# dselivanov/rsparse

Hardware: AMD Instinct MI355X
Metric: als_iterations_per_sec (higher is better)
Workload: dtype f32 (Gram products of rows > 512 / <= 32 non-zeros as 2 x fp16 / 3 x bf16 split terms of the fp32 operands, fp32 accumulate; everything else fp32); 1 GPU; WRMF implicit ALS, CG(3), synthetic 10000000x1000000, 500155883 nnz, rank 128, lambda 0.1; survey_config=3, feedback=implicit, n_items=1000000, nnz=500155883, rank=128, solver=conjugate_gradient, cg_steps=3, parallelism=rows sharded x1, factors replicated

## Files before the change

rsparse_amd/build.py:

```python
import subprocess
import sys
import time
from concurrent.futures import ThreadPoolExecutor
from pathlib import Path

PKG = Path(__file__).resolve().parent
CSRC = PKG / "csrc"
SRC = [CSRC / n for n in ("wrmf_kernels.hip", "wrmf_cgq.hip", "wrmf_cgp.hip", "wrmf_ne.hip", "wrmf_chol.hip", "wrmf_chol_wave.hip", "wrmf_chol_mf.hip", "wrmf_cg_mf.hip", "wrmf_chol_lr.hip",
                          "wrmf_topk.hip", "wrmf_topk_large.hip", "wrmf_similar.hip", "wrmf_metrics.hip", "wrmf_ingest.hip", "wrmf_nnls.hip", "wrmf_bias.hip", "wrmf_lu.hip",
                          "wrmf_f64.hip", "wrmf_wide.hip", "wrmf_wide_cg.hip", "wrmf_ctx_kernels.hip", "wrmf_schedule.cpp", "wrmf_capi.cpp", "wrmf_f64_capi.cpp", "wrmf_ctx.cpp")]
HEADERS = [CSRC / "wrmf_chol_mf.attrs.csv", CSRC / "wrmf_mf.h", CSRC / "wrmf_internal.h", CSRC / "wrmf_capi_common.h", CSRC / "wrmf_schedule.h", CSRC / "wrmf_device.h", CSRC / "wrmf_wave.h", CSRC / "wrmf_ldlt.h", CSRC / "wrmf_f64.h", PKG.parent / "include" / "rsparse_wrmf_hip.h"]
DEPS = SRC + HEADERS
OUT = PKG / "lib" / "librsparse_wrmf_hip.so"
FLAGS = ["--offload-arch=gfx950", "-O3", "-std=c++17", "-fPIC"]


EXTRA_FLAGS = {n: ["-mllvm", "-forceattrs-csv-path=" + str(CSRC / "wrmf_chol_mf.attrs.csv"), "-fno-slp-vectorize"] for n in ("wrmf_chol_mf.hip", "wrmf_cg_mf.hip")}
AUDITED = {"wrmf_chol_mf.hip", "wrmf_cg_mf.hip"}
REG_LIMIT = {"wrmf_cg_mf.hip": 512}


def audit_listing(src, extra, obj):
    sys.path.insert(0, str(PKG.parent / "tools" / "dbg"))
    import acc_audit
    lst = obj.with_suffix(".s")

    def listing(flags, floor):
        cmd = ["hipcc", *FLAGS, *flags, "-S", "--cuda-device-only", str(src), "-o", str(lst)]
        r = subprocess.run(cmd, stdout=subprocess.PIPE, stderr=subprocess.PIPE, text=True)
        if r.returncode != 0:
            raise RuntimeError("hipcc -S failed on %s:\n%s" % (src.name, r.stderr[-3000:]))
        acc, flight, _ = acc_audit.audit(str(lst), quiet=True, acc_floor=floor)
        return acc, flight, lst.read_text()
    acc, flight, text = listing(extra, 0)
# ... 23 lines not shown
    src = [s for s in SRC if s.exists()]
    hdr_m = max(h.stat().st_mtime for h in HEADERS)
    todo, objs = [], []
    for s in src:
        o = objdir / (s.stem + ".o")
        objs.append(o)
        if force or not o.exists() or o.stat().st_mtime < max(s.stat().st_mtime, hdr_m):
            todo.append((s, o))
    if not todo and out.exists() and all(out.stat().st_mtime >= o.stat().st_mtime for o in objs):
        return out

    def compile_one(so):
        s, o = so
        t0 = time.time()
        extra = EXTRA_FLAGS.get(s.name, [])
        cmd = ["hipcc", *FLAGS, *extra, "-c", str(s), "-o", str(o)]
        r = subprocess.run(cmd, stdout=subprocess.PIPE, stderr=subprocess.PIPE, text=True)
        if r.returncode != 0:
            raise RuntimeError("hipcc failed on %s:\n%s" % (s.name, r.stderr[-6000:]))
        if s.name in AUDITED:
            audit_listing(s, extra, o)
        if verbose:
            print("  %-20s %.1f s" % (s.name, time.time() - t0), flush=True)

    with ThreadPoolExecutor(max_workers=8) as ex:
        list(ex.map(compile_one, todo))
    cmd = ["hipcc", "--offload-arch=gfx950", "-fPIC", "-shared", *map(str, objs), "-ldl", "-lpthread", "-o", str(out)]
    subprocess.check_call(cmd)
    return out


if __name__ == "__main__":
    argv = sys.argv[1:]
    outp = argv[argv.index("--out") + 1] if "--out" in argv else None
# ... 3 lines not shown
```

rsparse_amd/csrc/wrmf_capi.cpp:

```cpp
#include "../../include/rsparse_wrmf_hip.h"

#include <cxxabi.h>

#include <algorithm>
#include <cfloat>
#include <cmath>
#include <cstdlib>
#include <cstring>
#include <string>
#include <vector>

#include "wrmf_capi_common.h"

using namespace rsparse_hip;

struct rsparse_hip_csc {
  DevCSC d;
  int device = 0;
  std::vector<void*> owned;
};

namespace {
thread_local std::string g_err;
}
// ... 119 lines not shown
}

int build_schedule(rsparse_hip_csc& m, const int32_t* host_col_ptrs) {
  DevCSC& d = m.d;
  int cus = 256;
  HIP_TRY(hipDeviceGetAttribute(&cus, hipDeviceAttributeMultiprocessorCount, m.device));
  d.q_cfg = cgq_default_cfg();
  SchedulePlan plan;
  if (!plan_schedule(host_col_ptrs, d.n_cols, cus, [](int len) { return cgq_bucket_of(len, cgq_default_cfg()); }, plan))
    return fail(RSPARSE_HIP_ERR_INVALID, "col_ptrs is not non-decreasing");
  d.max_len = plan.max_len; d.nnz_long = plan.nnz_long; d.n_empty = plan.n_empty;
  d.short_max = kTileNnz; d.n_long = plan.n_long;
  for (int b = 0; b < 7; b++) d.q_off[b] = plan.off[b];
  for (int b = 0; b < 6; b++) d.q_nnz[b] = plan.nnz[b];
  d.q_pair_first = plan.pair_first; d.q_team4_first = plan.team4_first;
  d.q_gt32 = plan.gt32; d.q_gt48 = plan.gt48; d.q_lr_first = plan.lr_first; d.q_n_lr = plan.n_lr;
  d.q_n_chol_long = plan.n_chol_long; d.q_n_nec = plan.n_nec;
  int rc;
  if ((rc = upload(m, plan.order, &d.q_order))) return rc;
  if ((rc = upload(m, plan.stream_off, &d.q_stream_off))) return rc;
  if ((rc = upload_cut(m, plan.cut, d.q_ne))) return rc;
  d.q_ne1 = d.q_ne;
  if ((rc = upload_deal(m, plan.fine, d.q_ne))) return rc;
  if ((rc = upload_deal(m, plan.coarse, d.q_ne1))) return rc;
  if (plan.nec_is_ne) {
    d.q_nec = d.q_ne;
  } else {
    if ((rc = upload_cut(m, plan.cut_nec, d.q_nec))) return rc;
    if ((rc = upload_deal(m, plan.nec, d.q_nec))) return rc;
  }
// ... 119 lines not shown
    hipError_t we = wave_cg ? launch_wide_cg_wave(a, implicit, kWideCgMaxLen, d.max_len > kWideCgMaxLen ? d.q_order : nullptr, 0, s)
                            : launch_als_wide(a, implicit, solver, g_ws.wide_m2, g_ws.wide_lu, s);
    if (we != hipSuccess) return hip_fail(we, wave_cg ? "launch_wide_cg_wave" : "launch_als_wide");
    if ((we = launch_sum_partials(g_ws.partials, wave_cg ? (size_t)grid_w : (size_t)grid, outw, s, g_ws.partials + g_ws.partial_slots())) != hipSuccess)
      return hip_fail(we, "launch_sum_partials");
    return RSPARSE_HIP_OK;
  }
  const bool cg = solver == RSPARSE_SOLVER_CONJUGATE_GRADIENT;
  const bool cgq = cg && use_cgq(rank, d_X, d_Y);
  QSchedule qs;
  qs.order = d.q_order;
  qs.cfg = d.q_cfg;
  qs.pair_first = d.q_pair_first;
  for (int b = 0; b < 7; b++) qs.off[b] = d.q_off[b];
  qs.team4_first = (implicit && bias && bias->gbias != 0.f) ? d.q_off[2] : d.q_team4_first;
  qs.pair_wide = cgp_wide_supported(rank, implicit, implicit && bias && bias->gbias != 0.f);
  const bool cg_mf = cgq && implicit && !bias && cg_mf_supported(rank, implicit) && d.q_order && d.q_off[1] > d.q_n_nec;
  if (cg_mf) {
    qs.mf_rows = d.q_order + d.q_n_nec;
    qs.mf_n = d.q_off[1] - d.q_n_nec;
  }
  const bool chol_mf = chol_mf_supported(rank) && !cg && solver == RSPARSE_SOLVER_CHOLESKY && !bias && d.q_order && ne_supported(rank) &&
                       use_cgq(rank, d_X, d_Y) && d.q_lr_first > d.q_off[1];
  const int mf_first = d.q_off[1];
  const int n_mf = chol_mf ? d.q_lr_first - mf_first : 0;
  const bool nec_lists = padded_rank(rank) > 64 && d.q_nec.wg > 0 && !chol_mf;
  const bool ne_chol = !cg && solver == RSPARSE_SOLVER_CHOLESKY && !bias && (nec_lists || d.q_ne.wg > 0 || chol_mf) &&
                       ne_supported(rank) && use_cgq(rank, d_X, d_Y);
  qs.ne = (cg_mf || (ne_chol && nec_lists)) ? d.q_nec : ((implicit && padded_rank(rank) == 128) ? d.q_ne : d.q_ne1);
  const size_t chol_base = chol2_loss_slots(d.n_cols);
// ... 1048 lines not shown
```

rsparse_amd/csrc/wrmf_cgq.hip:

```cpp
#include <algorithm>

#include "wrmf_internal.h"
#include "wrmf_device.h"

namespace rsparse_hip {
namespace {

using namespace dev;

constexpr int kGvFirstMinCapq = 16;
constexpr int kStreamPrefixQ = 4;
constexpr int kIdxPrefetchMaxWpr = 2;

constexpr int kMaxSavedSweeps = 4;

template <int KP>
struct QG {
  static constexpr int RPN = KP / 16;
  static constexpr int VW = RPN >= 4 ? 4 : RPN;
  static constexpr int NV = RPN / VW;
  __device__ static __forceinline__ int elem(int i, int r) { return (r / VW) * (16 * VW) + i * VW + (r % VW); }
};

template <int VW>
struct Piece;
template <>
struct Piece<4> { using type = float4; };
template <>
struct Piece<2> { using type = float2; };

__device__ __forceinline__ float groups_reduce_scatter4(const float a0, const float a1, const float a2, const float a3) {
  const auto s01 = __builtin_amdgcn_permlane16_swap(__float_as_uint(a0), __float_as_uint(a1), false, false);
  const float c = __uint_as_float(s01[0]) + __uint_as_float(s01[1]);
  const auto s23 = __builtin_amdgcn_permlane16_swap(__float_as_uint(a2), __float_as_uint(a3), false, false);
  const float d = __uint_as_float(s23[0]) + __uint_as_float(s23[1]);
  const auto t = __builtin_amdgcn_permlane32_swap(__float_as_uint(c), __float_as_uint(d), false, false);
  return __uint_as_float(t[0]) + __uint_as_float(t[1]);
}
template <int KP, int CAPQ, int WAVES, int WPR, int STREAM, bool IMPLICIT, int DMF = 0>
struct QSmem {
  static constexpr size_t gram_floats = (IMPLICIT && DMF != 1) ? (size_t)KP * KP : 0;
  static constexpr size_t vec_floats = IMPLICIT ? (size_t)WAVES * KP : 0;
  static constexpr size_t red_floats = WPR > 1 ? (size_t)2 * WAVES * KP + 2 * WAVES : 0;
  static constexpr bool cv_lds = !STREAM && CAPQ * (KP / 16) > 128;
  static constexpr size_t tsv_floats = (STREAM && !IMPLICIT) ? 0 : (size_t)WAVES * (cv_lds ? 3 : 2) * CAPQ * 4;
  static constexpr size_t pre_floats = STREAM ? (size_t)WAVES * kStreamPrefixQ * 4 * KP : 0;
  static constexpr int dmf_ps = KP + 8, dmf_os = KP + 4;
  static constexpr size_t dmf_floats = DMF ? (size_t)WAVES * dmf_ps + (size_t)WAVES * dmf_os : 0;
  static constexpr size_t pfx_floats =
      (!STREAM && WPR > kIdxPrefetchMaxWpr && (CAPQ == 16 || CAPQ == 20)) ? (size_t)WAVES * 2 * CAPQ * 4 : 0;
  static constexpr size_t wl_floats = cv_lds ? (size_t)WAVES * 2 : 0;
  static constexpr size_t xs_floats = cv_lds ? (size_t)WAVES * KP : 0;
  static constexpr size_t bytes =
      (gram_floats + vec_floats + red_floats + tsv_floats + pre_floats + dmf_floats + pfx_floats + wl_floats + xs_floats) * 4 + 16;
};

template <int KP, int CAPQ, int WAVES, int WPR, int STREAM, bool IMPLICIT, int DMF = 0, bool GB = false, bool KFULL = false>
__global__ __launch_bounds__(WAVES * 64, 2) void als_cgq_kernel(AlsArgs a, const int32_t* __restrict__ rows, int n_rows,
                                                             int rows_per_team, size_t loss_slot0) {
  using G_ = QG<KP>;
  constexpr int RPN = G_::RPN, VW = G_::VW, NV = G_::NV, CAP = CAPQ * 4, TEAMS = WAVES / WPR;
  using piece_t = typename Piece<VW>::type;
  using SM = QSmem<KP, CAPQ, WAVES, WPR, STREAM, IMPLICIT, DMF>;
  static_assert(WAVES % WPR == 0, "teams must tile the workgroup");
  constexpr bool GRS = RPN == 8 && VW == 4;
// ... 96 lines not shown
          split_f16(g0 * gs, g1 * gs, hi[e / 2], lo[e / 2]);
        }
        const uint4 h4 = {hi[0], hi[1], hi[2], hi[3]}, l4 = {lo[0], lo[1], lo[2], lo[3]};
        if constexpr (DMF == 1) {
          gAh[t][ks] = __builtin_bit_cast(f16x8, h4);
          gAl[t][ks] = __builtin_bit_cast(f16x8, l4);
        } else {
          *reinterpret_cast<uint4*>(sGf + ((t * 4 + ks) * 2 + 0) * 1024 + lane * 16) = h4;
          *reinterpret_cast<uint4*>(sGf + ((t * 4 + ks) * 2 + 1) * 1024 + lane * 16) = l4;
        }
      }
    if constexpr (DMF == 2) wave_sync();
  }
  float* vec = sVec + wv * KP;
  constexpr bool CVLDS = SM::cv_lds;
  float* tacc = sTsv + wv * (CVLDS ? 3 : 2) * CAP;
  float* tcur = tacc + CAP;
  float* csv = tcur + CAP;
  int buf = 0;
  double wloss = 0.0;
  double* wl_lds = reinterpret_cast<double*>(sPfx + SM::pfx_floats) + wv;
  if (CVLDS && lane == 0) *wl_lds = 0.0;
  float* xs = sPfx + SM::pfx_floats + SM::wl_floats + wv * KP;
  int pf_id = 0, pf_cnt = -1;
  float pf_c = 0.f;
  const int team_global = blockIdx.x * TEAMS + team;
  const int total_teams = gridDim.x * TEAMS;

  auto row_index = [&](int itn) { return team_global + itn * total_teams; };
  int row_c = 0, p1_c = 0, p2_c = 0, row_n = 0;
  if (rows_per_team > 0 && row_index(0) < n_rows) {
    row_c = rows[row_index(0)];
    p1_c = a.col_ptrs[row_c];
    p2_c = a.col_ptrs[row_c + 1];
  }
  if (rows_per_team > 1 && row_index(1) < n_rows) row_n = rows[row_index(1)];
  for (int it = 0; it < rows_per_team; ++it) {
    const int ri = row_index(it);
    const bool have = ri < n_rows;
    if (WPR == 1 && !DMF && !have) break;
    const int row = have ? rfl(row_c) : 0;
    const int p1 = have ? rfl(p1_c) : 0;
    const int p2 = have ? rfl(p2_c) : 0;
    {
      int p1_n = 0, p2_n = 0, row_nn = 0;
      if (it + 1 < rows_per_team && row_index(it + 1) < n_rows) {
        p1_n = a.col_ptrs[row_n];
        p2_n = a.col_ptrs[row_n + 1];
      }
      if (it + 2 < rows_per_team && row_index(it + 2) < n_rows) row_nn = rows[row_index(it + 2)];
      row_c = row_n;
      p1_c = p1_n;
      p2_c = p2_n;
      row_n = row_nn;
    }
    const int cnt = p2 - p1;
    float* yrow = a.Y + (size_t)row * k;
    if (!GB && WPR == 1 && cnt <= 0) {
      if (!DMF || have)
        for (int e = lane; e < k; e += 64) yrow[e] = 0.f;
      if constexpr (!DMF) continue;
    }
    constexpr int PQ = STREAM ? kStreamPrefixQ : 0, PCAP = PQ * 4, PTEAM = PCAP * WPR;
    const int pre = STREAM ? min(cnt, PTEAM) : 0;
    const int pw = STREAM ? max(0, min(PCAP, pre - tw * PCAP)) : 0;
    const int nchunks = (cnt - pre + CAP - 1) / CAP;
    constexpr bool resident = STREAM == 0;
    const float lam_use =
        IMPLICIT ? 0.f : (float)(a.lambda_loss * (a.dynamic_lambda ? (double)(float)cnt : 1.0));

    float* tscr = nullptr;
    float alph[kMaxSavedSweeps];
#pragma unroll
    for (int s2 = 0; s2 < kMaxSavedSweeps; s2++) alph[s2] = 0.f;
    if constexpr (STREAM == 1) {
      if (a.tscr && have && a.cg_steps <= kMaxSavedSweeps) tscr = a.tscr + a.stream_off[ri];
    }

    float xt[CAPQ][RPN];
    float cv[CVLDS ? 1 : CAPQ];
    constexpr int NSL = (CAP + 63) / 64;
    float cl[CVLDS ? 1 : NSL];
#pragma unroll
    for (int s2 = 0; s2 < (CVLDS ? 1 : NSL); s2++) cl[s2] = 0.f;
    auto csv_fill = [&](auto&& conf_of, const int n) {
#pragma unroll
      for (int s2 = 0; s2 < NSL; s2++) {
        const int sl = lane + 64 * s2;
        if (s2 == 0 || sl < CAP) csv[(sl & 3) * CAPQ + (sl >> 2)] = sl < n ? conf_of(sl) : 0.f;
      }
    };
    int ccnt = 0;

    constexpr bool ZPAD = STREAM == 0;
    constexpr bool TSAVE = STREAM == 0;
    constexpr bool GVFIRST = STREAM == 0 && CAPQ >= kGvFirstMinCapq;
    constexpr bool IDXPF = CAP <= 64 && ((STREAM == 0 && WPR <= kIdxPrefetchMaxWpr) || (STREAM == 1 && IMPLICIT));
    constexpr bool DMAPF = KFULL && !IDXPF && SM::pfx_floats > 0;
    int* pfxI = reinterpret_cast<int*>(sPfx) + wv * 2 * CAP;
    float* pfxC = sPfx + wv * 2 * CAP + CAP;
    auto dma_slot = [&](const int j0, const int n) {
      const int j = j0 + min(lane, n - 1);
      dma4(a.row_idx + j, lds_addr(pfxI));
      dma4(a.vals + j, lds_addr(pfxC));
      if constexpr (CAP > 64) {
        if (lane < CAP - 64) {
          const int j2 = j0 + min(lane + 64, n - 1);
          dma4(a.row_idx + j2, lds_addr(pfxI + 64));
          dma4(a.vals + j2, lds_addr(pfxC + 64));
        }
      }
    };
    int pf_pos = -1;
    auto gather_q = [&](auto nq_tag, const int base, const int n, const bool from_pf = false) {
      constexpr int NQG = decltype(nq_tag)::value;
      int id[NQG > 0 ? NQG : 1];
      if constexpr (DMAPF) {
        if (!from_pf && n > 0) {
          dma_slot(base, n);
          wait_vm<0>();
        }
        wave_sync();
#pragma unroll
        for (int q = 0; q < NQG; q++) {
          const int j = max(min(4 * q + g, n - 1), 0);
          id[q] = pfxI[j];
          if constexpr (!CVLDS) cv[q] = (!ZPAD || 4 * q + g < n) ? pfxC[j] : 0.f;
        }
        if constexpr (CVLDS) {
          csv_fill([&](int sl) { return pfxC[sl]; }, n);
        } else if constexpr (TSAVE) {
#pragma unroll
          for (int s2 = 0; s2 < NSL; s2++) cl[s2] = lane + 64 * s2 < n ? pfxC[min(lane + 64 * s2, CAP - 1)] : 0.f;
        }
        wave_sync();
      } else if (IDXPF && from_pf) {
        int* xi = reinterpret_cast<int*>(tacc);
        wave_sync();
        xi[lane & (CAP - 1)] = pf_id;
        tcur[lane & (CAP - 1)] = pf_c;
        wave_sync();
#pragma unroll
        for (int q = 0; q < NQG; q++) {
          const int j = max(min(4 * q + g, n - 1), 0);
          id[q] = xi[j];
          if constexpr (!CVLDS) cv[q] = (!ZPAD || 4 * q + g < n) ? tcur[j] : 0.f;
        }
        if constexpr (TSAVE) cl[0] = lane < n ? pf_c : 0.f;
        wave_sync();
      } else {
#pragma unroll
        for (int q = 0; q < NQG; q++) {
          const int j = max(min(4 * q + g, n - 1), 0);
          id[q] = a.row_idx[base + j];
          if constexpr (!CVLDS) {
            const float c = a.vals[base + j];
            cv[q] = (!ZPAD || 4 * q + g < n) ? c : 0.f;
          }
        }
        if constexpr (CVLDS) {
          wave_sync();
          csv_fill([&](int sl) { return a.vals[base + sl]; }, n);
          wave_sync();
        } else if constexpr (TSAVE) {
#pragma unroll
          for (int s2 = 0; s2 < NSL; s2++) cl[s2] = lane + 64 * s2 < n ? a.vals[base + lane + 64 * s2] : 0.f;
        }
      }
#pragma unroll
      for (int q = 0; q < NQG; q++) {
        const float* src = (!ZPAD || 4 * q + g < n) ? a.X + (size_t)id[q] * k : a.zero_row;
#pragma unroll
        for (int b = 0; b < NV; b++) {
          const int off = b * 16 * VW + i * VW;
          if constexpr (KFULL) {
            const piece_t pc = *reinterpret_cast<const piece_t*>(src + off);
            const float* pf = reinterpret_cast<const float*>(&pc);
#pragma unroll
            for (int c = 0; c < VW; c++) xt[q][b * VW + c] = pf[c];
          } else {
            const piece_t pc = *reinterpret_cast<const piece_t*>(src + min(off, k - VW));
            const float* pf = reinterpret_cast<const float*>(&pc);
#pragma unroll
            for (int c = 0; c < VW; c++) xt[q][b * VW + c] = off < k ? pf[c] : 0.f;
          }
        }
      }
    };
    auto gather = [&](const int base, const int n, const bool from_pf = false) {
      gather_q(std::integral_constant<int, CAPQ>{}, base, n, from_pf);
    };
    float* pre_lds = sPre + (size_t)wv * PQ * 4 * KP + g * KP;
    auto prefix_chunk = [&](const bool first) {
      if constexpr (PQ > 0) {
        const int base = p1 + tw * PCAP;
        if (first) {
          gather_q(std::integral_constant<int, PQ>{}, base, pw);
#pragma unroll
          for (int q = 0; q < PQ; q++)
#pragma unroll
            for (int b = 0; b < NV; b++) {
              piece_t pc;
              float* pf = reinterpret_cast<float*>(&pc);
// ... 218 lines not shown
                  const float* pf = reinterpret_cast<const float*>(&pc);
#pragma unroll
                  for (int c = 0; c < VW; c++) acc[b * VW + c] = fmaf(vv[u], pf[c], acc[b * VW + c]);
                }
              }
            }
          }
        };
        if constexpr (GVFIRST) dense_part();
        if (resident) {
          if (mode != 2 || !TSAVE) {
            quad_pass(v, mode, acc, lacc, nullptr);
          } else {
            wave_sync();
            float esum = 0.f;
#pragma unroll
            for (int s2 = 0; s2 < NSL; s2++) {
              const int sl = NSL == 1 ? (lane & (CAP - 1)) : min(lane + 64 * s2, CAP - 1);
              const float t = tacc[sl];
              const float clv = CVLDS ? csv[(sl & 3) * CAPQ + (sl >> 2)] : cl[s2];
              const float d = IMPLICIT ? ltgt - t : clv - t;
              const float e = IMPLICIT ? clv * d * d : d * d;
              esum += lane + 64 * s2 < ccnt ? e : 0.f;
            }
            lacc = row16_sum(esum);
          }
        } else if (mode == 2 && tscr) {
          for (int ch = tw; ch < (cnt + CAP - 1) / CAP; ch += WPR) {
            const int n = min(CAP, cnt - ch * CAP);
            if (lane < n) {
              const size_t pos = (size_t)ch * CAP + lane;
              float t = tscr[pos];
#pragma unroll
              for (int s2 = 0; s2 < kMaxSavedSweeps; s2++)
                if (s2 < a.cg_steps) t = fmaf(alph[s2], tscr[(size_t)(s2 + 1) * a.stream_nnz + pos], t);
              const float c = a.vals[p1 + pos];
              const float d = IMPLICIT ? ltgt - t : c - t;
              lacc += IMPLICIT ? c * d * d : d * d;
// ... 135 lines not shown
    float dummy = 0.f;
    sweep(x, 0, r, dummy, live);
    auto x_piece = [&](const int b) { return reinterpret_cast<piece_t*>(xs + b * 16 * VW + i * VW); };
    if constexpr (CVLDS) {
      if (g == 0) {
#pragma unroll
        for (int b = 0; b < NV; b++) {
          piece_t pc;
          float* pf = reinterpret_cast<float*>(&pc);
#pragma unroll
          for (int c = 0; c < VW; c++) pf[c] = x[b * VW + c];
          *x_piece(b) = pc;
        }
      }
    }
    if constexpr (IDXPF && STREAM == 0) {
      if (it + 1 < rows_per_team && row_index(it + 1) < n_rows) {
        const int np1 = rfl(p1_c), ncnt = rfl(p2_c) - np1;
        const int nper = min(CAP, (((ncnt + WPR - 1) / WPR) + 15) & ~15);
        const int ncc = max(0, min(nper, ncnt - tw * nper));
        if (ncc > 0) {
          const int j = np1 + tw * nper + min(lane & (CAP - 1), ncc - 1);
          pf_id = a.row_idx[j];
          pf_c = a.vals[j];
          pf_cnt = ncc;
        }
      }
    }
    if constexpr (DMAPF) {
      if (it + 1 < rows_per_team && row_index(it + 1) < n_rows) {
// ... 9 lines not shown
#pragma unroll
    for (int rr = 0; rr < RPN; rr++) p[rr] = r[rr];
    float rsold = dot16(r, r);
    bool conv = false;
    for (int itc = 0; itc < a.cg_steps; ++itc) {
      if (WPR == 1 && !DMF && conv) break;
      sweep(p, 1, ap, dummy, live && !conv, itc + 1);
      if (!conv) {
        const float pap = dot16(p, ap);
        const float alpha = (float)((double)rsold / (double)pap);
#pragma unroll
        for (int s2 = 0; s2 < kMaxSavedSweeps; s2++)
          if (s2 == itc) alph[s2] = alpha;
        if constexpr (TSAVE) {
          wave_sync();
#pragma unroll
          for (int s2 = 0; s2 < NSL; s2++) {
            const int sl = NSL == 1 ? (lane & (CAP - 1)) : lane + 64 * s2;
            if (CAP % 64 == 0 || sl < CAP) tacc[sl] = fmaf(alpha, tcur[sl], tacc[sl]);
          }
          wave_sync();
        }
        if constexpr (CVLDS) {
          if (g == 0) {
#pragma unroll
            for (int b = 0; b < NV; b++) {
              piece_t pc = *x_piece(b);
              float* pf = reinterpret_cast<float*>(&pc);
#pragma unroll
              for (int c = 0; c < VW; c++) pf[c] = fmaf(alpha, p[b * VW + c], pf[c]);
              *x_piece(b) = pc;
            }
          }
// ... 14 lines not shown
        }
      }
    }
    if constexpr (CVLDS) {
      wave_sync();
#pragma unroll
      for (int b = 0; b < NV; b++) {
        const piece_t pc = *x_piece(b);
        const float* pf = reinterpret_cast<const float*>(&pc);
#pragma unroll
        for (int c = 0; c < VW; c++) x[b * VW + c] = pf[c];
      }
    }
    float rl = 0.f;
    sweep(x, 2, ap, rl, live);
    if constexpr (DMAPF) wait_vm<0>();
    if constexpr (IDXPF && STREAM == 0) {
      asm volatile("" : "+v"(pf_id), "+v"(pf_c));
    }
    if (live && tw == 0) {
      const float xx = dot16(x, x);
      const double wl_row = IMPLICIT ? (double)rl + a.lambda_loss * (double)xx : (double)(rl + lam_use * xx);
      if constexpr (CVLDS) {
        if (lane == 0) *wl_lds += wl_row;
      } else {
        wloss += wl_row;
      }
      if (g == 0) {
#pragma unroll
        for (int b = 0; b < NV; b++) {
// ... 10 lines not shown
    }
  }
  if (lane == 0) a.loss_partials[loss_slot0 + (size_t)blockIdx.x * WAVES + wv] = CVLDS ? *wl_lds : wloss;
}

struct BucketDef { int waves, wpr, capq, stream, max_len; };
constexpr int kNB = 6;
constexpr int kNCfg = 2;
constexpr BucketDef kBuckets[kNCfg][kNB] = {
    {{8, 8, 16, 1, 0x7fffffff}, {8, 8, 16, 0, 512}, {4, 4, 16, 0, 256}, {4, 2, 16, 0, 128}, {4, 1, 16, 0, 64}, {4, 1, 8, 0, 32}},
    {{8, 8, 16, 1, 0x7fffffff}, {4, 4, 32, 0, 512}, {4, 2, 32, 0, 256}, {4, 1, 32, 0, 128}, {4, 1, 16, 0, 64}, {4, 1, 8, 0, 32}},
};
constexpr int cfg_of_kp(int KP) { return KP == 64 ? 1 : 0; }
constexpr int kTeam4Waves = 4, kTeam4Capq = 20;
static_assert(kTeam4Max == kTeam4Waves * kTeam4Capq * 4, "wrmf_internal.h's split and the kernel's capacity");
constexpr bool team4_split(int KP, bool GB) { return KP == 128 && !GB; }
int team4_first(const QSchedule& q) { return std::min(std::max(q.team4_first, q.off[1]), q.off[2]); }

template <int KP, int WAVES, int CAPQ, int WPR, int STREAM, bool IMPLICIT, bool GB, int DMF = 0, bool KFULL = false>
hipError_t launch_bucket(const AlsArgs& a, const int32_t* rows, int n_rows, int grid, size_t slot0, hipStream_t s,
                         hipEvent_t* ev_slot) {
  if (n_rows <= 0) return hipSuccess;
  constexpr bool kDmfGeometry = IMPLICIT && KP == 128 && WAVES == 4 && WPR == 1 && (CAPQ == 8 || CAPQ == 16) && STREAM == 0;
  if constexpr (kDmfGeometry && !DMF) {
    return launch_bucket<KP, WAVES, CAPQ, WPR, STREAM, IMPLICIT, GB, CAPQ == 8 ? 1 : 2>(a, rows, n_rows, grid, slot0, s, ev_slot);
  } else {
    if constexpr (!KFULL && STREAM == 0 && !(DMF == 1 && !GB)) {
      if (a.k == KP)
        return launch_bucket<KP, WAVES, CAPQ, WPR, STREAM, IMPLICIT, GB, DMF, true>(a, rows, n_rows, grid, slot0, s, ev_slot);
    }
    constexpr int TEAMS = WAVES / WPR;
    auto kern = als_cgq_kernel<KP, CAPQ, WAVES, WPR, STREAM, IMPLICIT, DMF, GB, KFULL>;
// ... 29 lines not shown
    return hipSuccess;
  }
};
thread_local BucketStreams g_bs;

int g_launch_mode = 2;
int concurrent_buckets() { return g_launch_mode; }

size_t bucket_slots(const QSchedule& q, int b, int k, bool implicit) {
  const int cfg = cfg_of_kp(padded_rank(k));
  const BucketDef d = kBuckets[cfg][b];
  if (d.wpr <= 0) return 0;
  if (d.stream && ne_supported(k)) return (size_t)(q.ne.entries + q.ne.nsplit) + (size_t)(q.mf_n > 0 ? cg_mf_loss_slots(q.mf_n) : 0);
  const int rows = q.off[b + 1] - q.off[b];
  if (b == 1 && padded_rank(k) == 128) {
    const int split = team4_first(q);
    return (size_t)cgq_bucket_grid(split - q.off[b], b, cfg) * d.waves + (size_t)cgq_team4_grid(q.off[b + 1] - split) * kTeam4Waves;
  }
  if (b == kNB - 1 && rows > 0 && cgp_supported(k, implicit)) {
    const int split = std::min(std::max(q.pair_first, q.off[b]), q.off[b + 1]);
    const size_t main = q.pair_wide ? (size_t)cgp_grid(split - q.off[b]) * 4 : (size_t)cgq_bucket_grid(split - q.off[b], b, cfg) * d.waves;
    return main + (size_t)cgp_grid(q.off[b + 1] - split) * 4;
  }
  return (size_t)cgq_bucket_grid(rows, b, cfg) * d.waves;
}

template <int KP, int CFG, bool IMPLICIT, bool GB>
hipError_t launch_all(const AlsArgs& a, const QSchedule& q, hipStream_t s, hipEvent_t* ev) {
  hipError_t err;
  size_t slot = 0;
  const int cmode = ev ? 0 : concurrent_buckets();
  const bool overlap = cmode != 0;
// ... 36 lines not shown
              ms = g_bs.st[B];                                                                              \
              if ((err = hipStreamWaitEvent(ms, g_bs.fork0, 0)) != hipSuccess) return err;                  \
            }                                                                                               \
            if ((err = launch_als_cg_mf(a, q.mf_rows, q.mf_n, (int)(slot + (size_t)(q.ne.entries + q.ne.nsplit)), ms, \
                                        ev ? ev + B : nullptr)) != hipSuccess)                              \
              return err;                                                                                   \
            if (mside) {                                                                                    \
              if ((err = hipEventRecord(g_bs.done[B], ms)) != hipSuccess) return err;                       \
              if ((err = hipStreamWaitEvent(s, g_bs.done[B], 0)) != hipSuccess) return err;                 \
            }                                                                                               \
          }                                                                                                 \
        } else if constexpr (D.stream && KP > 32) {        \
          return hipErrorInvalidValue;                                                                      \
        } else if constexpr (B == 1 && team4_split(KP, GB)) {                                              \
           \
          const int first = q.off[B], split = team4_first(q);                                               \
          const int n_main = split - first, n_t4 = q.off[B + 1] - split;                                    \
          const int g_main = cgq_bucket_grid(n_main, B, CFG);                                               \
          if ((err = launch_bucket<KP, D.waves, D.capq, D.wpr, D.stream, IMPLICIT, GB>(a, q.order + first, n_main, g_main, slot, \
                                                                                  bs, ev ? ev + B : nullptr)) != hipSuccess) \
            return err;                                                                                     \
          if ((err = launch_bucket<KP, kTeam4Waves, kTeam4Capq, kTeam4Waves, 0, IMPLICIT, GB>(              \
                   a, q.order + split, n_t4, cgq_team4_grid(n_t4), slot + (size_t)g_main * D.waves, bs,     \
                   n_main > 0 ? nullptr : (ev ? ev + B : nullptr))) != hipSuccess)                          \
            return err;                                                                                     \
        } else if (B == kNB - 1 && cgp_supported(a.k, IMPLICIT)) {                    \
           \
                                                 \
          const int first = q.off[B], split = std::min(std::max(q.pair_first, first), q.off[B + 1]);         \
          const int n_main = split - first, n_pair = q.off[B + 1] - split;                                   \
          size_t main_slots;                                                                                \
          if (q.pair_wide) {                                                                                \
            if ((err = launch_als_cgp(a, q.order + first, n_main, true, slot, bs, ev ? ev + B : nullptr)) != hipSuccess) \
              return err;                                                                                   \
            main_slots = (size_t)cgp_grid(n_main) * 4;                                                      \
          } else {                                                                                          \
            const int g_main = cgq_bucket_grid(n_main, B, CFG);                                             \
            if ((err = launch_bucket<KP, D.waves, D.capq, D.wpr, D.stream, IMPLICIT, GB>(a, q.order + first, n_main, g_main, slot, \
                                                                                    bs, ev ? ev + B : nullptr)) != hipSuccess) \
// ... 42 lines not shown
  const long per_wg = (long)teams * rows_per_team;
  long grid = (n_rows + per_wg - 1) / per_wg;
  if (grid < 1) grid = 1;
  return (int)grid;
}
}

int cgq_bucket_grid(int n_rows, int b, int cfg) {
  const BucketDef d = kBuckets[cfg][b];
  if (n_rows <= 0 || d.wpr <= 0) return 0;
  const int base = d.stream ? 16 : (d.wpr == 1 ? 64 : (d.wpr == 2 ? 64 : 32));
  return team_grid(n_rows, d.waves / d.wpr, base);
}

int cgq_team4_grid(int n_rows) { return n_rows <= 0 ? 0 : team_grid(n_rows, 1, 32); }

int cgq_bucket_of(int len, int cfg) {
  int best = 0;
  for (int b = 0; b < kNB; b++)
    if (kBuckets[cfg][b].wpr > 0 && len <= kBuckets[cfg][b].max_len) best = b;
  return best;
}

size_t cgq_loss_slots(const QSchedule& q, int k, bool implicit) {
  size_t n = 0;
  for (int b = 0; b < kNB; b++) n += bucket_slots(q, b, k, implicit);
  return n;
}

int cgq_default_cfg() { return 0; }
// ... 19 lines not shown
```

rsparse_amd/csrc/wrmf_internal.h:

```cpp
#pragma once
#include <hip/hip_runtime.h>
#include <cstdint>
#include <string>

#include "wrmf_schedule.h"

namespace rsparse_hip {

constexpr float kCgTol = 1e-10f;
constexpr double kCgTolD = 1e-10;
constexpr int kScdMaxIter = 10000;
constexpr float kScdTol = 1e-4f;
constexpr double kScdTolD = 1e-4;
constexpr float kNnlsEps = 1e-16f;
constexpr double kNnlsEpsD = 1e-16;

struct NeListSet {
  const int32_t* rows = nullptr;
  const int32_t* ptr = nullptr;
  int wg = 0;
  int entries = 0;
  const int32_t* segs = nullptr;
  int nseg = 0;
  const int32_t* split_rows = nullptr;
// ... 4 lines not shown
struct DevCSC {
  int n_rows = 0;
  int n_cols = 0;
  int64_t nnz = 0;
  const int32_t* col_ptrs = nullptr;
  const int32_t* row_idx = nullptr;
  const float* vals = nullptr;
  int n_long = 0;
  int short_max = 0;
  int max_len = 0;
  const int32_t* q_order = nullptr;
  int q_off[7] = {0, 0, 0, 0, 0, 0, 0};
  int q_cfg = 0;
  int q_pair_first = 0;
  int q_team4_first = 0;
  int64_t q_nnz[6] = {0, 0, 0, 0, 0, 0};
  const int64_t* q_stream_off = nullptr;
  int q_n_chol_long = 0;
  int q_gt32 = 0;
  int q_gt48 = 0;
  int q_lr_first = 0, q_n_lr = 0;
  NeListSet q_ne;
  NeListSet q_ne1;
  int q_n_nec = 0;
  NeListSet q_nec;
  int64_t nnz_long = 0;
  int n_empty = 0;
  mutable bool vals_frozen = false;
  mutable bool vstats_valid = false;
  mutable unsigned* vstats = nullptr;
// ... 46 lines not shown
  const int32_t* ne_segs;
  float* ne_seg_scratch;
  int* ne_seg_flags;
  int ne_chol;
  int ne_chol_min;
  const unsigned* ne_stats;
  const float* mf_XtX;
  const unsigned* wave_stats;
};

struct QSchedule {
  const int32_t* order;
  int off[7];
  int pair_first;
  int team4_first;
  bool pair_wide;
  int cfg;
  NeListSet ne;
  const int32_t* mf_rows = nullptr;
  int mf_n = 0;
};
int cgq_default_cfg();
void cgq_set_launch_mode(int mode);
int cgq_num_buckets();
int cgq_bucket_wpr(int cfg, int b);
int cgq_bucket_capq(int cfg, int b);
int cgq_bucket_waves(int cfg, int b);
int cgq_bucket_stream(int cfg, int b);
int cgq_bucket_grid(int n_rows, int bucket, int cfg);
int cgq_team4_grid(int n_rows);
int cgq_bucket_of(int len, int cfg);
size_t cgq_loss_slots(const QSchedule& q, int k, bool implicit);
bool cgp_supported(int k, bool implicit);
bool cgp_wide_supported(int k, bool implicit, bool gbias);
int cgp_grid(int n_rows);
hipError_t launch_als_cgp(const AlsArgs& a, const int32_t* rows, int n_rows, bool wide, size_t loss_slot0, hipStream_t s,
                          hipEvent_t* ev_slot);
bool ne_supported(int k);
constexpr int kNeMinLen = 512;
constexpr int kNeSegFloats = 4 * (11 * 16 * 64 + 128 + 2);
hipError_t launch_ne_stats(const float* X, int64_t nx, const float* vals, int64_t nnz, unsigned* stats, hipStream_t s,
                           const float* absmax_hint = nullptr, const unsigned* cached_vstats = nullptr,
                           unsigned* save_vstats = nullptr);
hipError_t launch_als_ne(const AlsArgs& a, const QSchedule& q, bool implicit, double* row_loss, hipStream_t s,
                         hipEvent_t* ev_slot = nullptr);
// ... 188 lines not shown
```

rsparse_amd/csrc/wrmf_schedule.cpp:

```cpp
#include "wrmf_schedule.h"

#include <algorithm>
#include <functional>
#include <queue>
#include <utility>

namespace rsparse_hip {

namespace {
int ne_slots(int cus) { return 2 * std::max(cus, 1); }
}

NeCut ne_cut(const int32_t* order, const int32_t* col_ptrs, int n_prefix, int64_t fixed, int cus) {
  NeCut c;
  if (n_prefix <= 0) return c;
  auto len_of = [&](int r) { return (int64_t)(col_ptrs[order[r] + 1] - col_ptrs[order[r]]); };
  auto steps_of = [](int64_t len) { return (len + 15) / 16; };
  const int n_slots = ne_slots(cus);
  int64_t total = 0;
  for (int r = 0; r < n_prefix; r++) total += steps_of(len_of(r)) + fixed;
  const int64_t share = std::max<int64_t>(1, total / n_slots);
  c.items.reserve((size_t)n_prefix + 64);
  int n_seg = 0;
  for (int r = 0; r < n_prefix; r++) {
// ... 63 lines not shown
    out.nec_is_ne = true;
    return true;
  }
  std::vector<int64_t> start((size_t)max_len + 2, 0);
  for (int i = 0; i < n; i++) start[(size_t)(max_len - (col_ptrs[i + 1] - col_ptrs[i])) + 1]++;
  int cnt_b[6] = {0, 0, 0, 0, 0, 0};
  for (int len = max_len; len >= 0; len--) {
    const int cnt = (int)start[(size_t)(max_len - len) + 1];
    if (!cnt) continue;
    if (len > kTileNnz) { out.n_long += cnt; out.nnz_long += (int64_t)len * cnt; }
    if (len == 0) out.n_empty += cnt;
    if (len > kCholLongLen) out.n_chol_long += cnt;
    if (len > kCgMfMax) out.n_nec += cnt;
    if (len > 16) out.pair_first += cnt;
    if (len > kTeam4Max) out.team4_first += cnt;
    if (len > 32) out.gt32 += cnt;
    if (len > 48) out.gt48 += cnt;
    if (len > kCholLrMax) out.lr_first += cnt;
    else if (len >= 1) out.n_lr += cnt;
    const int b = bucket_of(len);
    cnt_b[b] += cnt;
    out.nnz[b] += (int64_t)len * cnt;
  }
  for (int b = 0; b < 6; b++) out.off[b + 1] = out.off[b] + cnt_b[b];
  for (size_t b = 1; b < start.size(); b++) start[b] += start[b - 1];
  out.order.resize((size_t)n);
  for (int i = 0; i < n; i++) out.order[(size_t)start[(size_t)(max_len - (col_ptrs[i + 1] - col_ptrs[i]))]++] = i;
  const int n_stream = out.off[1];
  if (n_stream > 0) {
    out.stream_off.assign((size_t)n_stream + 1, 0);
// ... 18 lines not shown
```

rsparse_amd/csrc/wrmf_schedule.h:

```cpp
#pragma once
#include <cstdint>
#include <vector>

namespace rsparse_hip {

constexpr int kTileNnz = 32;
constexpr int kTeam4Max = 320;
constexpr int kCholLrMax = 64;
constexpr int kCholLongLen = 4096;
constexpr int kCgMfMax = 16384;
constexpr int kNeMaxSeg = 16;
constexpr int kNeMaxSegTotal = 1024;

struct NeCut {
  struct Item { int64_t cost; int32_t entry; };
  std::vector<Item> items;
  std::vector<int32_t> segs;
  std::vector<int32_t> split_rows;
  std::vector<int32_t> split_ptr;
  int nseg() const { return (int)(segs.size() / 6); }
};
struct NeDeal {
  std::vector<int32_t> rows, ptr;
  int wg() const { return ptr.empty() ? 0 : (int)ptr.size() - 1; }
};

NeCut ne_cut(const int32_t* order, const int32_t* col_ptrs, int n_prefix, int64_t fixed, int cus);
NeDeal ne_deal(const NeCut& cut, int n_prefix, int cus, bool fine);

struct SchedulePlan {
  int max_len = 0;
  int n_long = 0;
  int64_t nnz_long = 0;
  int n_empty = 0;
  std::vector<int32_t> order;
  int off[7] = {0, 0, 0, 0, 0, 0, 0};
  int64_t nnz[6] = {0, 0, 0, 0, 0, 0};
  int pair_first = 0;
  int team4_first = 0;
  int gt32 = 0, gt48 = 0;
  int lr_first = 0, n_lr = 0;
  int n_chol_long = 0;
  int n_nec = 0;
  std::vector<int64_t> stream_off;
  NeCut cut, cut_nec;
  NeDeal fine, coarse, nec;
  bool nec_is_ne = false;
};

bool plan_schedule(const int32_t* col_ptrs, int n_cols, int cus, int (*bucket_of)(int len), SchedulePlan& out);

}
```

Baseline: 8.334 iterations/s.

## Add a 4-wave team CG kernel for rows of 321-384 non-zeros

```diff
diff --git a/rsparse_amd/build.py b/rsparse_amd/build.py
--- a/rsparse_amd/build.py
+++ b/rsparse_amd/build.py
@@ -18,6 +18,37 @@
 EXTRA_FLAGS = {n: ["-mllvm", "-forceattrs-csv-path=" + str(CSRC / "wrmf_chol_mf.attrs.csv"), "-fno-slp-vectorize"] for n in ("wrmf_chol_mf.hip", "wrmf_cg_mf.hip")}
 AUDITED = {"wrmf_chol_mf.hip", "wrmf_cg_mf.hip"}
 REG_LIMIT = {"wrmf_cg_mf.hip": 512}
+NO_SPILL = {"wrmf_cgq.hip": ("14als_cgq_kernelILi128ELi24ELi4ELi4E",)}
+RESOURCE_FLAG = "-Rpass-analysis=kernel-resource-usage"
+
+
+def resource_violations(remarks, patterns, limit=256):
+    import re
+    rows, cur = [], None
+    for line in remarks.splitlines():
+        m = re.search(r"remark:\s+(.*?) \[-Rpass", line)
+        if not m:
+            continue
+        t = m.group(1).strip()
+        if t.startswith("Function Name:"):
+            cur = {"name": t.split(":", 1)[1].strip()}
+            rows.append(cur)
+        elif ":" in t and cur is not None:
+            k, v = t.rsplit(":", 1)
+            cur[k.strip()] = v.strip()
+    bad = []
+    for pat in patterns:
+        hit = [r for r in rows if pat in r["name"]]
+        if not hit:
+            bad.append((pat, "no such kernel in the compilation"))
+        for r in hit:
+            regs = int(r.get("VGPRs", "0")) + int(r.get("AGPRs", "0"))
+            for key in ("VGPRs Spill", "ScratchSize [bytes/lane]"):
+                if int(r.get(key, "0")):
+                    bad.append((r["name"], "%s = %s" % (key, r[key])))
+            if regs > limit:
+                bad.append((r["name"], "%d vector registers" % regs))
+    return bad
 
 
 def audit_listing(src, extra, obj):
@@ -71,10 +102,16 @@
         s, o = so
         t0 = time.time()
         extra = EXTRA_FLAGS.get(s.name, [])
-        cmd = ["hipcc", *FLAGS, *extra, "-c", str(s), "-o", str(o)]
+        guard = NO_SPILL.get(s.name)
+        cmd = ["hipcc", *FLAGS, *extra, *([RESOURCE_FLAG] if guard else []), "-c", str(s), "-o", str(o)]
         r = subprocess.run(cmd, stdout=subprocess.PIPE, stderr=subprocess.PIPE, text=True)
         if r.returncode != 0:
             raise RuntimeError("hipcc failed on %s:\n%s" % (s.name, r.stderr[-6000:]))
+        if guard:
+            bad = resource_violations(r.stderr, guard)
+            if bad:
+                o.unlink()
+                raise RuntimeError("%s: kernels that must not spill do:\n%s" % (s.name, "\n".join("  %s: %s" % b for b in bad)))
         if s.name in AUDITED:
             audit_listing(s, extra, o)
         if verbose:
diff --git a/rsparse_amd/csrc/wrmf_capi.cpp b/rsparse_amd/csrc/wrmf_capi.cpp
--- a/rsparse_amd/csrc/wrmf_capi.cpp
+++ b/rsparse_amd/csrc/wrmf_capi.cpp
@@ -157,6 +157,7 @@
   for (int b = 0; b < 7; b++) d.q_off[b] = plan.off[b];
   for (int b = 0; b < 6; b++) d.q_nnz[b] = plan.nnz[b];
   d.q_pair_first = plan.pair_first; d.q_team4_first = plan.team4_first;
+  d.q_team4_wide_first = plan.team4_wide_first;
   d.q_gt32 = plan.gt32; d.q_gt48 = plan.gt48; d.q_lr_first = plan.lr_first; d.q_n_lr = plan.n_lr;
   d.q_n_chol_long = plan.n_chol_long; d.q_n_nec = plan.n_nec;
   int rc;
@@ -306,6 +307,7 @@
   qs.pair_first = d.q_pair_first;
   for (int b = 0; b < 7; b++) qs.off[b] = d.q_off[b];
   qs.team4_first = (implicit && bias && bias->gbias != 0.f) ? d.q_off[2] : d.q_team4_first;
+  qs.team4_wide_first = (implicit && bias && bias->gbias != 0.f) ? d.q_off[2] : d.q_team4_wide_first;
   qs.pair_wide = cgp_wide_supported(rank, implicit, implicit && bias && bias->gbias != 0.f);
   const bool cg_mf = cgq && implicit && !bias && cg_mf_supported(rank, implicit) && d.q_order && d.q_off[1] > d.q_n_nec;
   if (cg_mf) {
diff --git a/rsparse_amd/csrc/wrmf_cgq.hip b/rsparse_amd/csrc/wrmf_cgq.hip
--- a/rsparse_amd/csrc/wrmf_cgq.hip
+++ b/rsparse_amd/csrc/wrmf_cgq.hip
@@ -37,18 +37,24 @@
   const auto t = __builtin_amdgcn_permlane32_swap(__float_as_uint(c), __float_as_uint(d), false, false);
   return __uint_as_float(t[0]) + __uint_as_float(t[1]);
 }
+template <bool ON>
+__device__ __forceinline__ int opaque_lane(int l) {
+  if constexpr (ON) asm volatile("" : "+v"(l));
+  return l;
+}
 template <int KP, int CAPQ, int WAVES, int WPR, int STREAM, bool IMPLICIT, int DMF = 0>
 struct QSmem {
   static constexpr size_t gram_floats = (IMPLICIT && DMF != 1) ? (size_t)KP * KP : 0;
   static constexpr size_t vec_floats = IMPLICIT ? (size_t)WAVES * KP : 0;
   static constexpr size_t red_floats = WPR > 1 ? (size_t)2 * WAVES * KP + 2 * WAVES : 0;
   static constexpr bool cv_lds = !STREAM && CAPQ * (KP / 16) > 128;
+  static constexpr bool wideq = !STREAM && CAPQ * (KP / 16) > 160;
   static constexpr size_t tsv_floats = (STREAM && !IMPLICIT) ? 0 : (size_t)WAVES * (cv_lds ? 3 : 2) * CAPQ * 4;
   static constexpr size_t pre_floats = STREAM ? (size_t)WAVES * kStreamPrefixQ * 4 * KP : 0;
   static constexpr int dmf_ps = KP + 8, dmf_os = KP + 4;
   static constexpr size_t dmf_floats = DMF ? (size_t)WAVES * dmf_ps + (size_t)WAVES * dmf_os : 0;
   static constexpr size_t pfx_floats =
-      (!STREAM && WPR > kIdxPrefetchMaxWpr && (CAPQ == 16 || CAPQ == 20)) ? (size_t)WAVES * 2 * CAPQ * 4 : 0;
+      (!STREAM && WPR > kIdxPrefetchMaxWpr && (CAPQ == 16 || CAPQ == 20 || CAPQ == 24)) ? (size_t)WAVES * 2 * CAPQ * 4 : 0;
   static constexpr size_t wl_floats = cv_lds ? (size_t)WAVES * 2 : 0;
   static constexpr size_t xs_floats = cv_lds ? (size_t)WAVES * KP : 0;
   static constexpr size_t bytes =
@@ -175,6 +181,7 @@
   }
   float* vec = sVec + wv * KP;
   constexpr bool CVLDS = SM::cv_lds;
+  constexpr bool WIDEQ = SM::wideq;
   float* tacc = sTsv + wv * (CVLDS ? 3 : 2) * CAP;
   float* tcur = tacc + CAP;
   float* csv = tcur + CAP;
@@ -203,18 +210,21 @@
     const int row = have ? rfl(row_c) : 0;
     const int p1 = have ? rfl(p1_c) : 0;
     const int p2 = have ? rfl(p2_c) : 0;
-    {
-      int p1_n = 0, p2_n = 0, row_nn = 0;
-      if (it + 1 < rows_per_team && row_index(it + 1) < n_rows) {
-        p1_n = a.col_ptrs[row_n];
-        p2_n = a.col_ptrs[row_n + 1];
-      }
-      if (it + 2 < rows_per_team && row_index(it + 2) < n_rows) row_nn = rows[row_index(it + 2)];
-      row_c = row_n;
-      p1_c = p1_n;
-      p2_c = p2_n;
-      row_n = row_nn;
-    }
+    constexpr bool META_LATE = WIDEQ && !KFULL;
+#define RSP_ADVANCE_META()                                                      \
+    {                                                                           \
+      int p1_n = 0, p2_n = 0, row_nn = 0;                                       \
+      if (it + 1 < rows_per_team && row_index(it + 1) < n_rows) {               \
+        p1_n = a.col_ptrs[row_n];                                               \
+        p2_n = a.col_ptrs[row_n + 1];                                           \
+      }                                                                         \
+      if (it + 2 < rows_per_team && row_index(it + 2) < n_rows) row_nn = rows[row_index(it + 2)]; \
+      row_c = row_n;                                                            \
+      p1_c = p1_n;                                                              \
+      p2_c = p2_n;                                                              \
+      row_n = row_nn;                                                           \
+    }
+    if constexpr (!META_LATE) RSP_ADVANCE_META()
     const int cnt = p2 - p1;
     float* yrow = a.Y + (size_t)row * k;
     if (!GB && WPR == 1 && cnt <= 0) {
@@ -245,9 +255,10 @@
 #pragma unroll
     for (int s2 = 0; s2 < (CVLDS ? 1 : NSL); s2++) cl[s2] = 0.f;
     auto csv_fill = [&](auto&& conf_of, const int n) {
+      const int ln = opaque_lane<WIDEQ>(lane);
 #pragma unroll
       for (int s2 = 0; s2 < NSL; s2++) {
-        const int sl = lane + 64 * s2;
+        const int sl = ln + 64 * s2;
         if (s2 == 0 || sl < CAP) csv[(sl & 3) * CAPQ + (sl >> 2)] = sl < n ? conf_of(sl) : 0.f;
       }
     };
@@ -273,6 +284,8 @@
       }
     };
     int pf_pos = -1;
+#define RSP_SLOT_IN(q, n) (SM::wideq ? g < (n) - 4 * (q) : 4 * (q) + g < (n))
+#define RSP_SLOT_J(q, n) max(SM::wideq ? min(g, (n) - 1 - 4 * (q)) + 4 * (q) : min(4 * (q) + g, (n) - 1), 0)
     auto gather_q = [&](auto nq_tag, const int base, const int n, const bool from_pf = false) {
       constexpr int NQG = decltype(nq_tag)::value;
       int id[NQG > 0 ? NQG : 1];
@@ -284,9 +297,9 @@
         wave_sync();
 #pragma unroll
         for (int q = 0; q < NQG; q++) {
-          const int j = max(min(4 * q + g, n - 1), 0);
+          const int j = RSP_SLOT_J(q, n);
           id[q] = pfxI[j];
-          if constexpr (!CVLDS) cv[q] = (!ZPAD || 4 * q + g < n) ? pfxC[j] : 0.f;
+          if constexpr (!CVLDS) cv[q] = (!ZPAD || RSP_SLOT_IN(q, n)) ? pfxC[j] : 0.f;
         }
         if constexpr (CVLDS) {
           csv_fill([&](int sl) { return pfxC[sl]; }, n);
@@ -303,20 +316,20 @@
         wave_sync();
 #pragma unroll
         for (int q = 0; q < NQG; q++) {
-          const int j = max(min(4 * q + g, n - 1), 0);
+          const int j = RSP_SLOT_J(q, n);
           id[q] = xi[j];
-          if constexpr (!CVLDS) cv[q] = (!ZPAD || 4 * q + g < n) ? tcur[j] : 0.f;
+          if constexpr (!CVLDS) cv[q] = (!ZPAD || RSP_SLOT_IN(q, n)) ? tcur[j] : 0.f;
         }
         if constexpr (TSAVE) cl[0] = lane < n ? pf_c : 0.f;
         wave_sync();
       } else {
 #pragma unroll
         for (int q = 0; q < NQG; q++) {
-          const int j = max(min(4 * q + g, n - 1), 0);
+          const int j = RSP_SLOT_J(q, n);
           id[q] = a.row_idx[base + j];
           if constexpr (!CVLDS) {
             const float c = a.vals[base + j];
-            cv[q] = (!ZPAD || 4 * q + g < n) ? c : 0.f;
+            cv[q] = (!ZPAD || RSP_SLOT_IN(q, n)) ? c : 0.f;
           }
         }
         if constexpr (CVLDS) {
@@ -328,12 +341,13 @@
           for (int s2 = 0; s2 < NSL; s2++) cl[s2] = lane + 64 * s2 < n ? a.vals[base + lane + 64 * s2] : 0.f;
         }
       }
+      const int ig = (SM::wideq && !KFULL) ? (opaque_lane<true>(lane) & 15) : i;
 #pragma unroll
       for (int q = 0; q < NQG; q++) {
-        const float* src = (!ZPAD || 4 * q + g < n) ? a.X + (size_t)id[q] * k : a.zero_row;
+        const float* src = (!ZPAD || RSP_SLOT_IN(q, n)) ? a.X + (size_t)id[q] * k : a.zero_row;
 #pragma unroll
         for (int b = 0; b < NV; b++) {
-          const int off = b * 16 * VW + i * VW;
+          const int off = b * 16 * VW + ig * VW;
           if constexpr (KFULL) {
             const piece_t pc = *reinterpret_cast<const piece_t*>(src + off);
             const float* pf = reinterpret_cast<const float*>(&pc);
@@ -348,6 +362,8 @@
         }
       }
     };
+#undef RSP_SLOT_IN
+#undef RSP_SLOT_J
     auto gather = [&](const int base, const int n, const bool from_pf = false) {
       gather_q(std::integral_constant<int, CAPQ>{}, base, n, from_pf);
     };
@@ -596,14 +612,15 @@
           } else {
             wave_sync();
             float esum = 0.f;
+            const int ln = opaque_lane<WIDEQ>(lane);
 #pragma unroll
             for (int s2 = 0; s2 < NSL; s2++) {
-              const int sl = NSL == 1 ? (lane & (CAP - 1)) : min(lane + 64 * s2, CAP - 1);
+              const int sl = NSL == 1 ? (lane & (CAP - 1)) : min(ln + 64 * s2, CAP - 1);
               const float t = tacc[sl];
               const float clv = CVLDS ? csv[(sl & 3) * CAPQ + (sl >> 2)] : cl[s2];
               const float d = IMPLICIT ? ltgt - t : clv - t;
               const float e = IMPLICIT ? clv * d * d : d * d;
-              esum += lane + 64 * s2 < ccnt ? e : 0.f;
+              esum += ln + 64 * s2 < ccnt ? e : 0.f;
             }
             lacc = row16_sum(esum);
           }
@@ -769,6 +786,8 @@
         }
       }
     }
+    if constexpr (META_LATE) RSP_ADVANCE_META()
+#undef RSP_ADVANCE_META
     if constexpr (IDXPF && STREAM == 0) {
       if (it + 1 < rows_per_team && row_index(it + 1) < n_rows) {
         const int np1 = rfl(p1_c), ncnt = rfl(p2_c) - np1;
@@ -808,9 +827,10 @@
           if (s2 == itc) alph[s2] = alpha;
         if constexpr (TSAVE) {
           wave_sync();
+          const int ln = opaque_lane<WIDEQ>(lane);
 #pragma unroll
           for (int s2 = 0; s2 < NSL; s2++) {
-            const int sl = NSL == 1 ? (lane & (CAP - 1)) : lane + 64 * s2;
+            const int sl = NSL == 1 ? (lane & (CAP - 1)) : ln + 64 * s2;
             if (CAP % 64 == 0 || sl < CAP) tacc[sl] = fmaf(alpha, tcur[sl], tacc[sl]);
           }
           wave_sync();
@@ -855,6 +875,7 @@
     }
     float rl = 0.f;
     sweep(x, 2, ap, rl, live);
+    if constexpr (META_LATE) p1_c = rfl(p1_c), p2_c = rfl(p2_c);
     if constexpr (DMAPF) wait_vm<0>();
     if constexpr (IDXPF && STREAM == 0) {
       asm volatile("" : "+v"(pf_id), "+v"(pf_c));
@@ -895,8 +916,13 @@
 constexpr int cfg_of_kp(int KP) { return KP == 64 ? 1 : 0; }
 constexpr int kTeam4Waves = 4, kTeam4Capq = 20;
 static_assert(kTeam4Max == kTeam4Waves * kTeam4Capq * 4, "wrmf_internal.h's split and the kernel's capacity");
+constexpr int kTeam4WideCapq = 24;
+static_assert(kTeam4WideMax == kTeam4Waves * kTeam4WideCapq * 4, "wrmf_schedule.h's split and the wide kernel's capacity");
+static_assert(kTeam4Max < kTeam4WideMax && kTeam4WideMax < 512, "the 4-wave launches take bucket 1's rows from its short end");
+static_assert(QSmem<128, kTeam4WideCapq, kTeam4Waves, kTeam4Waves, 0, true>::bytes <= 80 * 1024, "the wide team kernel's LDS");
 constexpr bool team4_split(int KP, bool GB) { return KP == 128 && !GB; }
 int team4_first(const QSchedule& q) { return std::min(std::max(q.team4_first, q.off[1]), q.off[2]); }
+int team4_wide_first(const QSchedule& q) { return std::min(std::max(q.team4_wide_first, q.off[1]), team4_first(q)); }
 
 template <int KP, int WAVES, int CAPQ, int WPR, int STREAM, bool IMPLICIT, bool GB, int DMF = 0, bool KFULL = false>
 hipError_t launch_bucket(const AlsArgs& a, const int32_t* rows, int n_rows, int grid, size_t slot0, hipStream_t s,
@@ -956,8 +982,9 @@
   if (d.stream && ne_supported(k)) return (size_t)(q.ne.entries + q.ne.nsplit) + (size_t)(q.mf_n > 0 ? cg_mf_loss_slots(q.mf_n) : 0);
   const int rows = q.off[b + 1] - q.off[b];
   if (b == 1 && padded_rank(k) == 128) {
-    const int split = team4_first(q);
-    return (size_t)cgq_bucket_grid(split - q.off[b], b, cfg) * d.waves + (size_t)cgq_team4_grid(q.off[b + 1] - split) * kTeam4Waves;
+    const int wide = team4_wide_first(q), split = team4_first(q);
+    return (size_t)cgq_bucket_grid(wide - q.off[b], b, cfg) * d.waves + (size_t)cgq_team4_wide_grid(split - wide) * kTeam4Waves +
+           (size_t)cgq_team4_grid(q.off[b + 1] - split) * kTeam4Waves;
   }
   if (b == kNB - 1 && rows > 0 && cgp_supported(k, implicit)) {
     const int split = std::min(std::max(q.pair_first, q.off[b]), q.off[b + 1]);
@@ -1024,15 +1051,21 @@
           return hipErrorInvalidValue;                                                                      \
         } else if constexpr (B == 1 && team4_split(KP, GB)) {                                              \
            \
-          const int first = q.off[B], split = team4_first(q);                                               \
-          const int n_main = split - first, n_t4 = q.off[B + 1] - split;                                    \
-          const int g_main = cgq_bucket_grid(n_main, B, CFG);                                               \
+           \
+          const int first = q.off[B], wide = team4_wide_first(q), split = team4_first(q);                   \
+          const int n_main = wide - first, n_w4 = split - wide, n_t4 = q.off[B + 1] - split;                \
+          const int g_main = cgq_bucket_grid(n_main, B, CFG), g_w4 = cgq_team4_wide_grid(n_w4);             \
           if ((err = launch_bucket<KP, D.waves, D.capq, D.wpr, D.stream, IMPLICIT, GB>(a, q.order + first, n_main, g_main, slot, \
                                                                                   bs, ev ? ev + B : nullptr)) != hipSuccess) \
             return err;                                                                                     \
+          if ((err = launch_bucket<KP, kTeam4Waves, kTeam4WideCapq, kTeam4Waves, 0, IMPLICIT, GB>(          \
+                   a, q.order + wide, n_w4, g_w4, slot + (size_t)g_main * D.waves, bs,                      \
+                   n_main > 0 ? nullptr : (ev ? ev + B : nullptr))) != hipSuccess)                          \
+            return err;                                                                                     \
           if ((err = launch_bucket<KP, kTeam4Waves, kTeam4Capq, kTeam4Waves, 0, IMPLICIT, GB>(              \
-                   a, q.order + split, n_t4, cgq_team4_grid(n_t4), slot + (size_t)g_main * D.waves, bs,     \
-                   n_main > 0 ? nullptr : (ev ? ev + B : nullptr))) != hipSuccess)                          \
+                   a, q.order + split, n_t4, cgq_team4_grid(n_t4),                                          \
+                   slot + (size_t)g_main * D.waves + (size_t)g_w4 * kTeam4Waves, bs,                        \
+                   n_main + n_w4 > 0 ? nullptr : (ev ? ev + B : nullptr))) != hipSuccess)                   \
             return err;                                                                                     \
         } else if (B == kNB - 1 && cgp_supported(a.k, IMPLICIT)) {                    \
            \
@@ -1105,6 +1138,7 @@
 }
 
 int cgq_team4_grid(int n_rows) { return n_rows <= 0 ? 0 : team_grid(n_rows, 1, 32); }
+int cgq_team4_wide_grid(int n_rows) { return cgq_team4_grid(n_rows); }
 
 int cgq_bucket_of(int len, int cfg) {
   int best = 0;
diff --git a/rsparse_amd/csrc/wrmf_internal.h b/rsparse_amd/csrc/wrmf_internal.h
--- a/rsparse_amd/csrc/wrmf_internal.h
+++ b/rsparse_amd/csrc/wrmf_internal.h
@@ -42,6 +42,7 @@
   int q_cfg = 0;
   int q_pair_first = 0;
   int q_team4_first = 0;
+  int q_team4_wide_first = 0;
   int64_t q_nnz[6] = {0, 0, 0, 0, 0, 0};
   const int64_t* q_stream_off = nullptr;
   int q_n_chol_long = 0;
@@ -118,6 +119,7 @@
   int off[7];
   int pair_first;
   int team4_first;
+  int team4_wide_first;
   bool pair_wide;
   int cfg;
   NeListSet ne;
@@ -133,6 +135,7 @@
 int cgq_bucket_stream(int cfg, int b);
 int cgq_bucket_grid(int n_rows, int bucket, int cfg);
 int cgq_team4_grid(int n_rows);
+int cgq_team4_wide_grid(int n_rows);
 int cgq_bucket_of(int len, int cfg);
 size_t cgq_loss_slots(const QSchedule& q, int k, bool implicit);
 bool cgp_supported(int k, bool implicit);
diff --git a/rsparse_amd/csrc/wrmf_schedule.cpp b/rsparse_amd/csrc/wrmf_schedule.cpp
--- a/rsparse_amd/csrc/wrmf_schedule.cpp
+++ b/rsparse_amd/csrc/wrmf_schedule.cpp
@@ -101,6 +101,7 @@
     if (len > kCgMfMax) out.n_nec += cnt;
     if (len > 16) out.pair_first += cnt;
     if (len > kTeam4Max) out.team4_first += cnt;
+    if (len > kTeam4WideMax) out.team4_wide_first += cnt;
     if (len > 32) out.gt32 += cnt;
     if (len > 48) out.gt48 += cnt;
     if (len > kCholLrMax) out.lr_first += cnt;
diff --git a/rsparse_amd/csrc/wrmf_schedule.h b/rsparse_amd/csrc/wrmf_schedule.h
--- a/rsparse_amd/csrc/wrmf_schedule.h
+++ b/rsparse_amd/csrc/wrmf_schedule.h
@@ -6,6 +6,7 @@
 
 constexpr int kTileNnz = 32;
 constexpr int kTeam4Max = 320;
+constexpr int kTeam4WideMax = 384;
 constexpr int kCholLrMax = 64;
 constexpr int kCholLongLen = 4096;
 constexpr int kCgMfMax = 16384;
@@ -38,6 +39,7 @@
   int64_t nnz[6] = {0, 0, 0, 0, 0, 0};
   int pair_first = 0;
   int team4_first = 0;
+  int team4_wide_first = 0;
   int gt32 = 0, gt48 = 0;
   int lr_first = 0, n_lr = 0;
   int n_chol_long = 0;
```

New measurement: 8.475 iterations/s, median of 6. 1.02x the previous value.
